# csteinmetz1/dasp-pytorch

Hardware: AMD Instinct MI355X
Metric: audio-samples/sec fwd+bwd, 6-band parametric_eq @ (256,2,131072) (higher is better)
Workload: dtype f32; 1 GPU; parametric_eq fwd+bwd (grad x + 18 controls) on (256,2,131072) fp32 per GPU, sr 44100, controls ~ U(ParametricEQ ranges); global_batch=256, parallelism=batch-shard x1, no collective, launch=eager, world_size=1

## Files before the change

dasp_pytorch_amd/csrc/sosfilt.hip:

```cpp
#include "common.hpp"
#include <type_traits>

#include "sos_tile.hpp"
#include <cstdlib>

namespace dasp {

__device__ __forceinline__ void nmul(double k, double p1, double q1, double p2, double q2, double& p, double& q) {
    p = p1 * p2 - k * q1 * q2;
    q = p1 * q2 + q1 * p2;
}
__device__ __forceinline__ void put_blk(float* o, double p, double q, double kap, int adj) {
    o[0] = (float)p;
    o[1] = (float)(adj ? -kap * q : q);
    o[2] = (float)(adj ? q : -kap * q);
    o[3] = (float)p;
}

struct D1 {
    double v, d;
};
__device__ __forceinline__ D1 dconst(double c) { return {c, 0.0}; }
__device__ __forceinline__ D1 operator+(D1 a, D1 b) { return {a.v + b.v, a.d + b.d}; }
__device__ __forceinline__ D1 operator-(D1 a, D1 b) { return {a.v - b.v, a.d - b.d}; }
__device__ __forceinline__ D1 operator*(D1 a, D1 b) { return {a.v * b.v, a.d * b.v + a.v * b.d}; }
__device__ __forceinline__ D1 operator/(D1 a, D1 b) {
    const double iv = 1.0 / b.v, q = a.v * iv;
    return {q, (a.d - q * b.d) * iv};
}
__device__ __forceinline__ D1 operator*(double c, D1 a) { return {c * a.v, c * a.d}; }
__device__ __forceinline__ D1 operator+(double c, D1 a) { return {c + a.v, a.d}; }
__device__ __forceinline__ D1 operator-(double c, D1 a) { return {c - a.v, -a.d}; }
__device__ __forceinline__ D1 operator-(D1 a) { return {-a.v, -a.d}; }
__device__ __forceinline__ D1 dsin(D1 a) { return {sin(a.v), cos(a.v) * a.d}; }
__device__ __forceinline__ D1 dcos(D1 a) { return {cos(a.v), -sin(a.v) * a.d}; }
__device__ __forceinline__ D1 dsqrt(D1 a) { const double r = sqrt(a.v); return {r, 0.5 / r * a.d}; }
__device__ __forceinline__ D1 dexp(D1 a) { const double e = exp(a.v); return {e, e * a.d}; }

struct PeqSpec {
    int types[8];
    double sample_rate;
    const float* rows[24];
    int norm;
    double lo[24], span[24];
    unsigned* flag;
};

__device__ void rbj_design(int type, double sample_rate, double gain_db, double fc, double qf, int dir, double* c5, double* dc5) {
    const D1 g = {gain_db, dir == 0 ? 1.0 : 0.0}, f = {fc, dir == 1 ? 1.0 : 0.0}, q = {qf, dir == 2 ? 1.0 : 0.0};
    const D1 A = dexp((2.302585092994045684 / 40.0) * g);
    const D1 w0 = (2.0 * 3.14159265358979323846 / sample_rate) * f;
    double sn, cs;
    sincos(w0.v, &sn, &cs);
    const D1 sw = {sn, cs * w0.d}, cw = {cs, -sn * w0.d};
    const D1 alpha = sw / (2.0 * q);
    const D1 sA = dsqrt(A);
    D1 b0, b1, b2, a0, a1, a2;
    if (type == 2) {
        b0 = A * ((A + dconst(1)) + (A - dconst(1)) * cw + 2.0 * (sA * alpha));
        b1 = -2.0 * (A * ((A - dconst(1)) + (A + dconst(1)) * cw));
        b2 = A * ((A + dconst(1)) + (A - dconst(1)) * cw - 2.0 * (sA * alpha));
        a0 = (A + dconst(1)) - (A - dconst(1)) * cw + 2.0 * (sA * alpha);
        a1 = 2.0 * ((A - dconst(1)) - (A + dconst(1)) * cw);
        a2 = (A + dconst(1)) - (A - dconst(1)) * cw - 2.0 * (sA * alpha);
    } else if (type == 1) {
        b0 = A * ((A + dconst(1)) - (A - dconst(1)) * cw + 2.0 * (sA * alpha));
        b1 = 2.0 * (A * ((A - dconst(1)) - (A + dconst(1)) * cw));
        b2 = A * ((A + dconst(1)) - (A - dconst(1)) * cw - 2.0 * (sA * alpha));
        a0 = (A + dconst(1)) + (A - dconst(1)) * cw + 2.0 * (sA * alpha);
        a1 = -2.0 * ((A - dconst(1)) + (A + dconst(1)) * cw);
        a2 = (A + dconst(1)) + (A - dconst(1)) * cw - 2.0 * (sA * alpha);
    } else if (type == 0) {
        b0 = 1.0 + alpha * A;
        b1 = -2.0 * cw;
        b2 = 1.0 - alpha * A;
        a0 = 1.0 + alpha / A;
        a1 = -2.0 * cw;
        a2 = 1.0 - alpha / A;
    } else if (type == 3) {
        b0 = 0.5 * (1.0 - cw);
        b1 = 1.0 - cw;
        b2 = 0.5 * (1.0 - cw);
        a0 = 1.0 + alpha;
        a1 = -2.0 * cw;
        a2 = 1.0 - alpha;
    } else {
        b0 = 0.5 * (1.0 + cw);
        b1 = -(1.0 + cw);
        b2 = 0.5 * (1.0 + cw);
        a0 = 1.0 + alpha;
        a1 = -2.0 * cw;
        a2 = 1.0 - alpha;
    }
    const D1 n[5] = {b0 / a0, b1 / a0, b2 / a0, a1 / a0, a2 / a0};
    for (int c = 0; c < 5; ++c) {
        c5[c] = n[c].v;
        dc5[c] = n[c].d;
    }
}

constexpr double OM_MIN = 1e-5;
#ifndef DASP_DF_OM_MIN
#define DASP_DF_OM_MIN 0.125
#endif
#ifndef DASP_STATES_CACHED
#define DASP_STATES_CACHED 1
#endif

template <int S>
__device__ __forceinline__ void section_coefs(const float* __restrict__ sos, const float* __restrict__ params, const PeqSpec& spec, int item, int k, int dir,
                                              bool report_range, double (&c5)[5], double (&dc5)[5], double& a0) {
    a0 = 1.0;
#pragma unroll
    for (int c = 0; c < 5; ++c) dc5[c] = 0.0;
    if (params && spec.norm) {
        const float* p = params + ((size_t)item * S + k) * 3;
        double v[3];
        for (int c = 0; c < 3; ++c) {
            const double pc = (double)p[c];
            if (report_range && spec.flag && (pc < 0.0 || pc > 1.0) && dir == 0) atomicOr(spec.flag, 1u << (3 * k + c));
            v[c] = spec.lo[3 * k + c] + spec.span[3 * k + c] * pc;
        }
        rbj_design(spec.types[k], spec.sample_rate, v[0], v[1], v[2], dir, c5, dc5);
        for (int c = 0; c < 5; ++c) dc5[c] *= spec.span[3 * k + dir];
    } else if (params) {
        const float* p = params + ((size_t)item * S + k) * 3;
        rbj_design(spec.types[k], spec.sample_rate, (double)p[0], (double)p[1], (double)p[2], dir, c5, dc5);
    } else if (!sos) {
        rbj_design(spec.types[k], spec.sample_rate, (double)spec.rows[3 * k][item], (double)spec.rows[3 * k + 1][item],
                   (double)spec.rows[3 * k + 2][item], dir, c5, dc5);
    } else {
        const float* sr = sos + ((size_t)item * S + k) * 6;
        a0 = (double)sr[3];
        c5[0] = sr[0] / a0; c5[1] = sr[1] / a0; c5[2] = sr[2] / a0; c5[3] = sr[4] / a0; c5[4] = sr[5] / a0;
    }
}

template <int S> struct GramFin;
template <int S, bool AGENT> __device__ __forceinline__ void gram_basis_responses(const double* cf, double* bas, int tid);
template <int S> __device__ __forceinline__ constexpr int basis_doubles();

template <int S, int L>
__global__ void __launch_bounds__(256)
sos_prep_kernel(const float* __restrict__ sos, const float* __restrict__ params, PeqSpec spec,
                float* __restrict__ tab, double* __restrict__ dtab, int nsq_seg = 0, double* __restrict__ segtab = nullptr,
                double* __restrict__ basis = nullptr, int nitems = 0) {
    using LY = SosLayout<S, L>;
    constexpr int S2 = 2 * S, NN = S2 * S2;
    __shared__ double sec[S][10];
    __shared__ double cfb[S][8];
    __shared__ double Phi[2][NN], T1[2][NN], T2[2][NN];
    __shared__ double vv[2][2][S2];
    if (basis && (int)blockIdx.x >= nitems) {
        const int it = blockIdx.x - nitems;
#ifdef DASP_TRACE
        if (it == 0 && threadIdx.x == 0) g_trace[48] = clock64();
#endif
        if (threadIdx.x < S) {
            double c5[5], dc5[5], a0;
            section_coefs<S>(sos, params, spec, it, threadIdx.x, 0, false, c5, dc5, a0);
            const double sg = -0.5 * c5[3];
            double om = sqrt(fabs(sg * sg - c5[4]));
            om = om < OM_MIN ? OM_MIN : om;
            for (int c = 0; c < 5; ++c) cfb[threadIdx.x][c] = c5[c];
            cfb[threadIdx.x][5] = sg; cfb[threadIdx.x][6] = om; cfb[threadIdx.x][7] = 1.0 / om;
        }
        __syncthreads();
#ifdef DASP_TRACE
        if (it == 0 && threadIdx.x == 0) g_trace[49] = clock64();
#endif
        gram_basis_responses<S, false>(&cfb[0][0], basis + (size_t)it * basis_doubles<S>(), threadIdx.x);
#ifdef DASP_TRACE
        asm volatile("s_waitcnt vmcnt(0)" ::: "memory");
        if (it == 0 && threadIdx.x == 0) g_trace[50] = clock64();
#endif
        return;
    }
    __shared__ float Gsh[2][L][S2];
    __shared__ double Pd[S][7][2];
    __shared__ float hsh[L];
    const int tid = threadIdx.x, item = blockIdx.x;
    PTRACE(40, 0);
    float* tb = tab + (size_t)item * LY::TOTAL;
    double* dt = dtab + (size_t)item * S * DT_STRIDE;

    if (tid < 4) tb[LY::CNT + tid] = 0.f;
    if (tid == 4) {
        const unsigned tg = ((unsigned)wall_clock64() * 2654435761u) ^ ((unsigned)item * 0x9E3779B1u);
        tb[LY::TAG] = __builtin_bit_cast(float, tg | 1u);
    }
    for (int e = tid; e < 2 * L * LY::YMC; e += 256) tb[LY::YM + e] = 0.f;
    if (tid < 3 * S) {
        const int k = tid / 3, dir = tid % 3;
        double c5[5], dc5[5], a0;
        section_coefs<S>(sos, params, spec, item, k, dir, true, c5, dc5, a0);
        double* d = dt + k * DT_STRIDE;
        for (int c = 0; c < 5; ++c) d[DT_J + c * 3 + dir] = dc5[c];
        if (dir == 0) {
            const double b0 = c5[0], b1 = c5[1], b2 = c5[2], a1 = c5[3], a2 = c5[4];
            const double sg = -0.5 * a1, disc = sg * sg - a2;
            const double kap = disc < 0 ? 1.0 : -1.0;
            double om = sqrt(fabs(disc));
            om = om < OM_MIN ? OM_MIN : om;
            const double g1 = b1 - b0 * a1, g2 = ((b2 - b0 * a2) + g1 * sg) / om;
            sec[k][0] = sg; sec[k][1] = om; sec[k][2] = kap * om; sec[k][3] = g1; sec[k][4] = g2; sec[k][5] = b0; sec[k][6] = kap;
            sec[k][7] = b1; sec[k][8] = b2;
            const bool direct = disc < 0 && om >= DASP_DF_OM_MIN && !(b0 == 1.0 && b1 == a1 && b2 == a2);
            float* df = tb + LY::DF + k * 8;
            df[0] = (float)b1; df[1] = (float)b2; df[2] = (float)-a1; df[3] = (float)-a2;
            df[4] = (float)(-g1 * sg + g2 * om); df[5] = (float)(-g1 * kap * om - g2 * sg); df[6] = (float)(1.0 / om); df[7] = (float)(sg / om);
            float* cf = tb + LY::COEF + k * 8;
            cf[0] = (float)sg; cf[1] = (float)om; cf[2] = (float)(kap * om); cf[3] = (float)g1; cf[4] = (float)g2;
            cf[5] = (float)b0; cf[6] = (float)kap; cf[7] = direct ? 1.f : 0.f;
            d[DT_OM] = direct ? 1.0 : om;
            for (int c = 0; c < 5; ++c) d[DT_B0 + c] = c5[c];
            d[DT_A0] = a0; d[7] = kap;
            d[23] = 0.0;
            d[DT_SG32] = (double)(float)sg; d[DT_NF] = direct ? 0.0 : 1.0; d[27] = 0.0;
        }
    }
    PTRACE(41, 0);
    __syncthreads();
    PTRACE(47, 0);
    for (int e = tid; e < 2 * NN; e += 256) {
        const int sys = e / NN, i = (e % NN) / S2, j = e % S2;
        const int kk = i / 2, r = i % 2, jj = j / 2, c = j % 2;
        const int fk = sys ? S - 1 - kk : kk, fj = sys ? S - 1 - jj : jj;
        const double sg = sec[fk][0], om = sec[fk][1], kom = sec[fk][2];
        const int rr = sys ? c : r, cc = sys ? r : c;
        const double a_el = rr == cc ? sg : (rr == 0 ? -kom : om);
        const double Bk = sys ? sec[fk][3 + r] : (r == 0 ? 1.0 : 0.0);
        const double Cj = sys ? (c == 0 ? 1.0 : 0.0) : sec[fj][3 + c];
        double gain = 1.0;
#pragma unroll
        for (int m = 0; m < S; ++m) {
            const double dm = sec[sys ? S - 1 - m : m][5];
            gain *= (m > jj && m < kk) ? dm : 1.0;
        }
        const double v = jj == kk ? a_el : (jj < kk ? Bk * gain * Cj : 0.0);
        Phi[sys][i * S2 + j] = v;
        T1[sys][i * S2 + j] = v;
        T2[sys][i * S2 + j] = 0.0;
    }
    PTRACE(46, 0);
    if (tid < 2 * S2) {
        const int sys = tid / S2, i = tid % S2, kk = i / 2, r = i % 2;
        const int fk = sys ? S - 1 - kk : kk;
        double gain = 1.0;
        for (int m = 0; m < kk; ++m) gain *= sec[sys ? S - 1 - m : m][5];
        vv[0][sys][i] = (sys ? sec[fk][3 + r] : (r == 0 ? 1.0 : 0.0)) * gain;
    }
    PTRACE(42, 0);
    __syncthreads();

    if (tid < 64) {
        for (int m = 0; m < L; ++m) {
            const int cur = m & 1;
            if (tid < 2 * S2) {
                const int sys = tid / S2, i = tid % S2;
                const double v = vv[cur][sys][i];
                Gsh[sys][m][i] = (float)v;
                double acc = 0.0;
                for (int j = 0; j < S2; ++j) acc += Phi[sys][i * S2 + j] * vv[cur][sys][j];
                vv[cur ^ 1][sys][i] = acc;
            }
            wave_lds_sync();
        }
    } else if (tid >= 128 && tid < 128 + 1 + S2) {
        const int ex = tid - 128, c0 = ex - 1;
        double s1[S], s2[S];
#pragma unroll
        for (int k = 0; k < S; ++k) { s1[k] = (c0 == 2 * k) ? 1.0 : 0.0; s2[k] = (c0 == 2 * k + 1) ? 1.0 : 0.0; }
        for (int n = 0; n < L; ++n) {
            double u = (ex == 0 && n == 0) ? 1.0 : 0.0;
#pragma unroll
            for (int k = 0; k < S; ++k) {
                const double sg = sec[k][0], om = sec[k][1], kom = sec[k][2], g1 = sec[k][3], g2 = sec[k][4], d = sec[k][5];
                const double o = d * u + g1 * s1[k] + g2 * s2[k];
                const double t1 = sg * s1[k] - kom * s2[k] + u;
                s2[k] = om * s1[k] + sg * s2[k];
                s1[k] = t1;
                u = o;
            }
            if (ex == 0) hsh[n] = (float)u;
            else tb[LY::YM + n * LY::YMC + L + state_pos<S>(c0)] = (float)u;
        }
    } else if (tid >= 192 && tid < 192 + S2) {
        const int c0 = tid - 192;
        double l1[S], l2[S];
#pragma unroll
        for (int i = 0; i < S; ++i) { l1[i] = (c0 == 2 * i) ? 1.0 : 0.0; l2[i] = (c0 == 2 * i + 1) ? 1.0 : 0.0; }
        for (int n = L - 1; n >= 0; --n) {
            double g = 0.0;
#pragma unroll
            for (int i = 0; i < S; ++i) {
                const int k = S - 1 - i;
                const double sg = sec[k][0], om = sec[k][1], kom = sec[k][2], g1 = sec[k][3], g2 = sec[k][4], d = sec[k][5];
                const double o = d * g + l1[i];
                const double t1 = sg * l1[i] + om * l2[i] + g1 * g;
                l2[i] = -kom * l1[i] + sg * l2[i] + g2 * g;
                l1[i] = t1;
                g = o;
            }
            tb[LY::YMA + n * LY::YMC + L + state_pos<S>(c0)] = (float)g;
        }
    } else if (tid < 128) {
        const int l = tid - 64;
        double (*src)[NN] = T1;
        double (*dst)[NN] = T2;
        for (int step = 1; step < L; step <<= 1) {
            constexpr int NTRI = S * (S + 1) / 2 * 4;
            for (int e = l; e < 2 * NTRI; e += 64) {
                const int sys = e / NTRI, q = e % NTRI, blk = q >> 2;
                const int kk = (blk >= 1) + (blk >= 3) + (blk >= 6) + (blk >= 10) + (blk >= 15) + (blk >= 21) + (blk >= 28);
                const int jj = blk - kk * (kk + 1) / 2;
                const int i = 2 * kk + ((q >> 1) & 1), j = 2 * jj + (q & 1);
                double acc = 0.0;
#pragma unroll
                for (int m = 0; m < S2; ++m) acc += src[sys][i * S2 + m] * src[sys][m * S2 + j];
                dst[sys][i * S2 + j] = acc;
            }
            wave_lds_sync();
            double (*tmp)[NN] = src; src = dst; dst = tmp;
        }
        for (int e = l; e < 2 * S * S * 4; e += 64) {
            const int sys = e / (S * S * 4), k = (e / (S * 4)) % S, j = (e / 4) % S, c = e % 4;
            tb[(sys ? LY::MCA : LY::MC) + (k * S + j) * 4 + c] = (float)src[sys][(2 * k + (c & 1)) * S2 + 2 * j + (c >> 1)];
        }
        if (l < S) {
            const int k = l;
            const double kap = sec[k][6];
            double p = src[0][(2 * k) * S2 + 2 * k], q = src[0][(2 * k + 1) * S2 + 2 * k];
            for (int lv = 0; lv < 7; ++lv) {
                Pd[k][lv][0] = p; Pd[k][lv][1] = q;
                if (lv < 4) {
                    put_blk(tb + LY::PL + (k * 4 + lv) * 4, p, q, kap, 0);
                    put_blk(tb + LY::PLA + ((S - 1 - k) * 4 + lv) * 4, p, q, kap, 1);
                }
                if (lv == 6) {
                    put_blk(tb + LY::P64 + k * 4, p, q, kap, 0);
                    put_blk(tb + LY::P64A + (S - 1 - k) * 4, p, q, kap, 1);
                }
                double p2, q2;
                nmul(kap, p, q, p, q, p2, q2);
                p = p2; q = q2;
            }
        }
    }
    PTRACE(43, 0); PTRACE(44, 64);
    __syncthreads();
    for (int e = tid; e < L * L; e += 256) {
        const int n = e / L, j = e % L;
        if (j <= n) tb[LY::YM + n * LY::YMC + j] = hsh[n - j];
        else tb[LY::YMA + n * LY::YMC + j] = hsh[j - n];
        if (j == n) tb[LY::YMA + n * LY::YMC + j] = hsh[0];
    }
    for (int e = tid; e < 2 * L * S2; e += 256) {
        const int sys = e / (L * S2), m = (e / S2) % L, i = e % S2;
        if (sys == 0) tb[LY::GT + ((i >> 1) * L + (L - 1 - m)) * 2 + (i & 1)] = Gsh[0][m][i];
        else tb[LY::GAT + ((i >> 1) * L + m) * 2 + (i & 1)] = Gsh[1][m][i];
    }
    for (int e = tid; e < S * 64; e += 256) {
        const int k = e / 64, c = e % 64, m = c + 1;
        const double kap = sec[k][6];
        double p = 1.0, q = 0.0;
        for (int l = 0; l < 7; ++l)
            if (m & (1 << l)) {
                double p2, q2;
                nmul(kap, p, q, Pd[k][l][0], Pd[k][l][1], p2, q2);
                p = p2; q = q2;
            }
        put_blk(tb + LY::PW + (k * 64 + c) * 4, p, q, kap, 0);
        put_blk(tb + LY::PWA + ((S - 1 - k) * 64 + c) * 4, p, q, kap, 1);
    }
    PTRACE(45, 0);
    if (segtab) {
        constexpr int NTRI = S * (S + 1) / 2 * 4;
        int nl = 0;
        for (int v = L; v > 1; v >>= 1) ++nl;
        double (*src)[NN] = (nl & 1) ? T2 : T1;
        double (*dst)[NN] = (nl & 1) ? T1 : T2;
        for (int step = 0; step < nsq_seg; ++step) {
            for (int e = tid; e < 2 * NTRI; e += 256) {
                const int sys = e / NTRI, q = e % NTRI, blk = q >> 2;
                const int kk = (blk >= 1) + (blk >= 3) + (blk >= 6) + (blk >= 10) + (blk >= 15) + (blk >= 21) + (blk >= 28);
                const int jj = blk - kk * (kk + 1) / 2;
                const int i = 2 * kk + ((q >> 1) & 1), j = 2 * jj + (q & 1);
                double acc = 0.0;
#pragma unroll
                for (int m = 0; m < S2; ++m) acc += src[sys][i * S2 + m] * src[sys][m * S2 + j];
                dst[sys][i * S2 + j] = acc;
            }
            __syncthreads();
            double (*tmp)[NN] = src; src = dst; dst = tmp;
        }
        for (int e = tid; e < 2 * NN; e += 256) segtab[(size_t)item * 2 * NN + e] = src[e / NN][e % NN];
    }
}

__device__ __forceinline__ void seg_state_store(float* p, f2 v) {
    __hip_atomic_store(p, v.x, __ATOMIC_RELAXED, __HIP_MEMORY_SCOPE_AGENT);
    __hip_atomic_store(p + 1, v.y, __ATOMIC_RELAXED, __HIP_MEMORY_SCOPE_AGENT);
}
template <int S, int W>
__device__ __forceinline__ void chain_by_last_workgroup(int* __restrict__ cnt, int n_wg, const double* __restrict__ Phi, const float* z,
                                                        float* __restrict__ start, int row0, int nrows, int G, int adjoint,
                                                        float* __restrict__ scratch , int scratch_stride) {
    constexpr int S2 = 2 * S, GB = 64;
    __shared__ int s_last;
    __shared__ double s_st[W][2][S2];
    asm volatile("s_waitcnt vmcnt(0)" ::: "memory");
    __syncthreads();
    if (threadIdx.x == 0) {
        s_last = handoff_arrive_is_last(cnt, n_wg);
    }
    __syncthreads();
    if (!s_last) return;
    const int l = lane_id(), w = wave_id();
    float* zs = scratch + w * scratch_stride;
    double prow[S2];
#pragma unroll
    for (int j = 0; j < S2; ++j) prow[j] = l < S2 ? Phi[l * S2 + j] : 0.0;
    const int first = adjoint ? G - 1 : 0, step = adjoint ? -1 : 1;
    for (int row = row0 + w; row < row0 + nrows; row += W) {
        if (l < S2) {
            s_st[w][0][l] = 0.0;
            start[((size_t)row * G + first) * S2 + l] = 0.f;
        }
        int cur = 0;
        for (int n0 = 0; n0 < G - 1; n0 += GB) {
            const int nblk = G - 1 - n0 < GB ? G - 1 - n0 : GB;
            wave_lds_sync();
            for (int e = l; e < nblk * S2; e += 64) {
                const int g = first + (n0 + e / S2) * step;
                zs[e] = __hip_atomic_load(z + ((size_t)row * G + g) * S2 + e % S2, __ATOMIC_RELAXED, __HIP_MEMORY_SCOPE_AGENT);
            }
            wave_lds_sync();
            for (int i = 0; i < nblk; ++i) {
                const int g = first + (n0 + i) * step;
                if (l < S2) {
                    double acc = (double)zs[i * S2 + l];
#pragma unroll
                    for (int j = 0; j < S2; ++j) acc += prow[j] * s_st[w][cur][j];
                    s_st[w][cur ^ 1][l] = acc;
                    start[((size_t)row * G + g + step) * S2 + l] = (float)acc;
                }
                wave_lds_sync();
                cur ^= 1;
            }
        }
    }
}


__device__ __forceinline__ void lookback_publish(unsigned long long* w, float v, unsigned tag) {
    __hip_atomic_store(w, ((unsigned long long)tag << 32) | __builtin_bit_cast(unsigned, v), __ATOMIC_RELAXED, __HIP_MEMORY_SCOPE_AGENT);
}
template <int S, int W>
__device__ __forceinline__ void lookback_start(const unsigned long long* z64, int seg, int G, int order, const double* __restrict__ Phi, unsigned tag,
                                               float* inbox, int seq, float* zs ,
                                               double (*st)[2 * S] , unsigned* err, int family) {
    constexpr int S2 = 2 * S, GB = 64;
    const int l = lane_id(), w = wave_id();
    const int npred = order > 0 ? seg : G - 1 - seg, first = order > 0 ? 0 : G - 1;
    double prow[S2];
#pragma unroll
    for (int j = 0; j < S2; ++j) prow[j] = w == 0 && l < S2 && npred > 0 ? Phi[l * S2 + j] : 0.0;
    if (w == 0 && l < S2) st[0][l] = 0.0;
    int cur = 0;
    __syncthreads();
    for (int n0 = 0; n0 < npred; n0 += GB) {
        const int nblk = npred - n0 < GB ? npred - n0 : GB;
        if (n0) __syncthreads();
        for (int e = threadIdx.x; e < nblk * S2; e += 64 * W) {
            const unsigned long long* wp = z64 + (size_t)(first + order * (n0 + e / S2)) * S2 + e % S2;
            zs[e] = lookback_poll(wp, tag, err, family);
        }
        __syncthreads();
        if (w == 0) {
            for (int i = 0; i < nblk; ++i) {
                if (l < S2) {
                    double acc = (double)zs[i * S2 + l];
#pragma unroll
                    for (int j = 0; j < S2; ++j) acc += prow[j] * st[cur][j];
                    st[cur ^ 1][l] = acc;
                }
                wave_lds_sync();
                cur ^= 1;
            }
        }
    }
    if (w == 0) {
        wave_lds_sync();
        if (l < S2) inbox[4 * (l >> 1) + (l & 1)] = (float)st[cur][l];
        if (l < S) inbox[4 * l + 2] = __builtin_bit_cast(float, seq);
    }
}

template <int S, int L, int W, int SEG = 0>
__global__ void __launch_bounds__(64 * W, W >= 16 ? 4 : (W * 2 + 3) / 4)
sos_fwd_kernel(const float* __restrict__ tab, int tab_bcast, const float* __restrict__ x, float* __restrict__ y,
               float* __restrict__ carries, int C, int N, int nt, int vec,
               int G = 1, int Tseg = 0, const float* __restrict__ segstart = nullptr, float* __restrict__ zseg = nullptr,
               float* __restrict__ chain_tab = nullptr, const double* __restrict__ segtab = nullptr, float* __restrict__ chain_start = nullptr,
               unsigned* __restrict__ err = nullptr) {
    using LY = SosLayout<S, L>;
    constexpr int S2 = 2 * S, TS = 64 * L, IMG = 64 * L;
    constexpr int LDS_T = W * 2 * IMG, LDS_MB = W * S * 4, LDS_PW = S * 64 * 4;
    __shared__ __attribute__((aligned(16))) float lds[LDS_T + LDS_MB + LDS_PW];
    const int lane = lane_id(), wave = wave_id();
    const int row = SEG ? blockIdx.x / G : blockIdx.x, seg = SEG ? blockIdx.x % G : 0;
    const int t0 = SEG ? seg * Tseg : 0, t1 = SEG ? (t0 + Tseg < nt ? t0 + Tseg : nt) : nt;
    const float* __restrict__ tb = tab + (size_t)(tab_bcast ? 0 : row / C) * LY::TOTAL;
    const float* __restrict__ xr = x + (size_t)row * N;
    float* __restrict__ yr = y + (size_t)row * N;
    const int mb_in = wave * S * 4, mb_out = ((wave + 1) % W) * S * 4;
    float* pw_lds = lds + LDS_MB;
    float* tbx = pw_lds + LDS_PW + wave * 2 * IMG;
    float* tby = tbx + IMG;
    if (SEG) {
        for (int i = threadIdx.x; i < LDS_MB; i += 64 * W) {
            float v = 0.f;
            if (i < S * 4) {
                const int comp = i & 3;
                if (comp == 2) v = __builtin_bit_cast(float, t0);
                else if (SEG == 1 && comp < 2) v = segstart[((size_t)row * G + seg) * S2 + 2 * (i >> 2) + comp];
            }
            lds[i] = v;
        }
    } else {
        for (int i = threadIdx.x; i < LDS_MB; i += 64 * W) lds[i] = 0.f;
    }
    for (int i = threadIdx.x; i < LDS_PW; i += 64 * W) pw_lds[i] = tb[LY::PW + i];
    __syncthreads();
    const f4* pws = reinterpret_cast<const f4*>(pw_lds);

    f2 Kreg[S];
#pragma unroll
    for (int k = 0; k < S; ++k) Kreg[k] = f2{0.f, 0.f};
    const unsigned a_x = __builtin_amdgcn_readfirstlane(lds_addr(tbx));
    float Aop[4];
    chunk_table_operands<S, L>(tb + LY::GT, Aop, lane);
    static_assert(L == 16 && S2 <= 16, "one 16 x 16 output block per 16 chunks");
    float AT[4], AO[4];
    if (SEG != 2) cascade_map_operands<S, L>(tb + LY::YM, LY::YMC, AT, AO, lane);
    const unsigned tag = SEG == 3 ? __builtin_amdgcn_readfirstlane(__builtin_bit_cast(unsigned, tb[LY::TAG])) : 0u;
    unsigned long long* z64 = reinterpret_cast<unsigned long long*>(zseg) + (size_t)row * G * S2;

    auto sweep = [&](auto scan_tag, const int seq0, const bool first_tile_requested = false) {
        constexpr bool SCAN = decltype(scan_tag)::value;
        if (!first_tile_requested && t0 + wave < t1 && tile_full<L>((long)(t0 + wave) * TS, N, vec)) tile_dma_issue_swz(xr + (size_t)(t0 + wave) * TS, a_x, lane);
        int stores_in_flight = 0;
        for (int t = t0 + wave; t < t1; t += W) {
            int toff = 0;
            asm volatile("" : "+s"(toff));
            const float* __restrict__ tbl = tb + toff;
            const bool full = tile_full<L>((long)t * TS, N, vec);
            WIDE_PRIO(DASP_SCAN_PRIO);
            TRACE(0);
            if (full) wait_vmcnt(stores_in_flight);
            else tile_global_to_swz_guarded(tbx, xr, (long)t * TS, N);
            f4 Bop[4], zacc[4];
            chunk_products_load(tbx, Bop, lane);
            pin(Bop);
            if (t + W < t1 && tile_full<L>((long)(t + W) * TS, N, vec)) tile_dma_issue_swz(xr + (size_t)(t + W) * TS, a_x, lane);
            TRACE(1);
            float Z[L];
            chunk_products_issue(Bop, Aop, zacc);
            chunk_products_collect<L>(tby, zacc, Z, lane, lane);
            pin(Z); TRACE(5);

            f2 st[S];
            MboxPeek pk;
            SCAN_PRIO(DASP_SCAN_PRIO);
            tile_scan<S, L>(Z, [](f2 v) { return v; }, st, tbl + LY::MC, tbl + LY::PL, tbl + LY::P64, pws, lane,
                [&](int k) { if (W > 1) pk = mbox_peek(lds, mb_in + 4 * k); },
                [&](int k, f2& K) {
                    if (W == 1) K = Kreg[k];
                    else if (pk.seq == t + seq0) K = f2{pk.a, pk.b};
                    else { float a, b; mbox_wait(lds, mb_in + 4 * k, t + seq0, a, b); K = f2{a, b}; }
                },
                [&](int k, f2 Kn) {
                    if (W == 1) Kreg[k] = f2{read_lane(Kn.x, 63), read_lane(Kn.y, 63)};
                    else if (t + 1 < t1) mbox_publish<63>(lds, mb_out + 4 * k, Kn.x, Kn.y, t + 1 + seq0);
                    else if (SCAN && lane == 63) {
                        if (SEG == 3) { lookback_publish(z64 + (size_t)seg * S2 + 2 * k, Kn.x, tag); lookback_publish(z64 + (size_t)seg * S2 + 2 * k + 1, Kn.y, tag); }
                        else seg_state_store(zseg + ((size_t)row * G + seg) * S2 + 2 * k, Kn);
                    }
                }
#ifdef DASP_TRACE
                , blockIdx.x == 7 && threadIdx.x == 64 && t >= 40 && t < 40 + W
#endif
                );
            SCAN_PRIO(0);
            TRACE(2);
            if (SCAN) {
                stores_in_flight = 0;
                continue;
            }
            if (carries) {
                static_assert(S % 2 == 0, "states are stored in section pairs");
                f4* cs = reinterpret_cast<f4*>(carries) + ((size_t)row * nt + t) * (S / 2) * 64 + lane;
#pragma unroll
                for (int m = 0; m < S / 2; ++m) {
                    const f4 v = f4{st[2 * m].x, st[2 * m].y, st[2 * m + 1].x, st[2 * m + 1].y};
                    if (DASP_FWD_NT & 4) st_stream(cs + m * 64, v); else cs[m * 64] = v;
                }
            }

            f4 yacc[4];
            cascade_outputs_mfma_acc<S, L>(tby, st, Bop, AT, AO, lane, yacc);
            TRACE(3);
            WIDE_PRIO(DASP_SCAN_PRIO);
            if (DASP_DIRECT_OUT && full) {
                mfma_granules_to_global(yr + (size_t)t * TS, yacc, DASP_FWD_NT & 2, lane);
            } else {
                mfma_granules_to_image(tby, yacc, lane);
                if (full) tile_swz_to_global_full(tby, yr, (long)t * TS, DASP_FWD_NT & 2, lane);
                else tile_swz_to_global_guarded(tby, yr, (long)t * TS, N);
            }
            stores_in_flight = full ? (carries ? S / 2 : 0) + L / 4 : -1;
            TRACE(4);
        }
    };
    if (SEG == 3) {
        sweep(std::true_type{}, 0);
        constexpr int SEQ2 = 1 << 28;
        __shared__ double lb_st[2][S2];
        if (t0 + wave < t1 && tile_full<L>((long)(t0 + wave) * TS, N, vec)) tile_dma_issue_swz(xr + (size_t)(t0 + wave) * TS, a_x, lane);
        lookback_start<S, W>(z64, seg, G, 1, segtab + (size_t)(tab_bcast ? 0 : row / C) * 2 * S2 * S2, tag, lds, t0 + SEQ2, pw_lds + LDS_PW + IMG, lb_st, err, DASP_DEVERR_SOS_FWD);
        __syncthreads();
        sweep(std::false_type{}, SEQ2, true);
    } else if (SEG == 2) {
        sweep(std::true_type{}, 0);
    } else {
        sweep(std::false_type{}, 0);
    }
    if (SEG == 2 && chain_tab) {
        const int item = tab_bcast ? 0 : row / C;
        chain_by_last_workgroup<S, W>(reinterpret_cast<int*>(chain_tab + (size_t)item * LY::TOTAL + LY::CNT) + 1, tab_bcast ? (int)gridDim.x : C * G,
                                      segtab + (size_t)item * 2 * S2 * S2, zseg, chain_start, tab_bcast ? 0 : item * C,
                                      tab_bcast ? (int)gridDim.x / G : C, G, 0, pw_lds + LDS_PW, 2 * IMG);
    }
}

#include "sos_gram_fin.hpp"

template <int S, int L, int W, int SEG = 0>
__global__ void __launch_bounds__(64 * W, (W * 2 + 3) / 4)
sos_bwd_kernel(const float* __restrict__ tab, int tab_bcast, const float* __restrict__ gy, float* __restrict__ gx, int C, int N, int nt, int vec,
               int G = 1, int Tseg = 0, const float* __restrict__ segstart = nullptr, float* __restrict__ zseg = nullptr,
               float* __restrict__ chain_tab = nullptr, const double* __restrict__ segtab = nullptr, float* __restrict__ chain_start = nullptr) {
    using LY = SosLayout<S, L>;
    constexpr bool GX = SEG != 2;
    constexpr int S2 = 2 * S, TS = 64 * L, IMG = 64 * L, REGION = 2 * IMG;
    constexpr int LDS_T = W * REGION, LDS_MB = W * S * 4, LDS_PW = S * 64 * 4, LDS_CF = S * 16;
    __shared__ __attribute__((aligned(16))) float lds[LDS_T + LDS_MB + LDS_PW + LDS_CF];
    const int lane = lane_id(), wave = wave_id();
    const int row = SEG ? blockIdx.x / G : blockIdx.x, seg = SEG ? blockIdx.x % G : 0;
    const int t0 = SEG ? seg * Tseg : 0, t1 = SEG ? (t0 + Tseg < nt ? t0 + Tseg : nt) : nt, nr = t1 - t0;
    const float* __restrict__ tb = tab + (size_t)(tab_bcast ? 0 : row / C) * LY::TOTAL;
    const float* __restrict__ gr = gy + (size_t)row * N;
    float* __restrict__ gxr = gx + (size_t)row * N;
    const int mb_in = wave * S * 4, mb_out = ((wave + 1) % W) * S * 4;
    float* cf_lds = lds + LDS_MB;
    float* pw_lds = cf_lds + LDS_CF;
    float* tbg = pw_lds + LDS_PW + wave * REGION;
    float* tbo = tbg + IMG;
    for (int i = threadIdx.x; i < LDS_MB; i += 64 * W) {
        float v = 0.f;
        if (i < S * 4) {
            const int comp = i & 3;
            if (comp == 2) v = __builtin_bit_cast(float, t1);
            else if (SEG == 1 && comp < 2) v = segstart[((size_t)row * G + seg) * S2 + 2 * (i >> 2) + comp];
        }
        lds[i] = v;
    }
    for (int i = threadIdx.x; i < LDS_PW; i += 64 * W) pw_lds[i] = tb[LY::PWA + i];
    for (int i = threadIdx.x; i < S * 8; i += 64 * W) cf_lds[i] = tb[LY::COEF + i];
    for (int i = threadIdx.x; i < S * 8; i += 64 * W) cf_lds[S * 8 + i] = tb[LY::DF + i];
// ... 927 lines not shown
```

Before: 192.0 billion channel-samples/s.

## Restructure sos prep kernel to overlap per-wave table writes and drop a barrier

```diff
diff --git a/dasp_pytorch_amd/csrc/sosfilt.hip b/dasp_pytorch_amd/csrc/sosfilt.hip
--- a/dasp_pytorch_amd/csrc/sosfilt.hip
+++ b/dasp_pytorch_amd/csrc/sosfilt.hip
@@ -146,7 +146,7 @@
                 float* __restrict__ tab, double* __restrict__ dtab, int nsq_seg = 0, double* __restrict__ segtab = nullptr,
                 double* __restrict__ basis = nullptr, int nitems = 0) {
     using LY = SosLayout<S, L>;
-    constexpr int S2 = 2 * S, NN = S2 * S2;
+    constexpr int S2 = 2 * S, NN = S2 * S2, NTRI = S * (S + 1) / 2 * 4;
     __shared__ double sec[S][10];
     __shared__ double cfb[S][8];
     __shared__ double Phi[2][NN], T1[2][NN], T2[2][NN];
@@ -190,6 +190,7 @@
         tb[LY::TAG] = __builtin_bit_cast(float, tg | 1u);
     }
     for (int e = tid; e < 2 * L * LY::YMC; e += 256) tb[LY::YM + e] = 0.f;
+    for (int e = tid; e < 2 * NN; e += 256) { (&Phi[0][0])[e] = 0.0; (&T1[0][0])[e] = 0.0; (&T2[0][0])[e] = 0.0; }
     if (tid < 3 * S) {
         const int k = tid / 3, dir = tid % 3;
         double c5[5], dc5[5], a0;
@@ -222,9 +223,11 @@
     PTRACE(41, 0);
     __syncthreads();
     PTRACE(47, 0);
-    for (int e = tid; e < 2 * NN; e += 256) {
-        const int sys = e / NN, i = (e % NN) / S2, j = e % S2;
-        const int kk = i / 2, r = i % 2, jj = j / 2, c = j % 2;
+    for (int e = tid; e < 2 * NTRI; e += 256) {
+        const int sys = e / NTRI, q = e % NTRI, blk = q >> 2;
+        const int kk = (blk >= 1) + (blk >= 3) + (blk >= 6) + (blk >= 10) + (blk >= 15) + (blk >= 21) + (blk >= 28);
+        const int jj = blk - kk * (kk + 1) / 2;
+        const int r = (q >> 1) & 1, c = q & 1, i = 2 * kk + r, j = 2 * jj + c;
         const int fk = sys ? S - 1 - kk : kk, fj = sys ? S - 1 - jj : jj;
         const double sg = sec[fk][0], om = sec[fk][1], kom = sec[fk][2];
         const int rr = sys ? c : r, cc = sys ? r : c;
@@ -237,79 +240,136 @@
             const double dm = sec[sys ? S - 1 - m : m][5];
             gain *= (m > jj && m < kk) ? dm : 1.0;
         }
-        const double v = jj == kk ? a_el : (jj < kk ? Bk * gain * Cj : 0.0);
+        const double v = jj == kk ? a_el : Bk * gain * Cj;
         Phi[sys][i * S2 + j] = v;
         T1[sys][i * S2 + j] = v;
-        T2[sys][i * S2 + j] = 0.0;
     }
     PTRACE(46, 0);
-    if (tid < 2 * S2) {
-        const int sys = tid / S2, i = tid % S2, kk = i / 2, r = i % 2;
+    if (tid >= 192 && tid < 192 + 2 * S2) {
+        const int t3 = tid - 192, sys = t3 / S2, i = t3 % S2, kk = i / 2, r = i % 2;
         const int fk = sys ? S - 1 - kk : kk;
         double gain = 1.0;
-        for (int m = 0; m < kk; ++m) gain *= sec[sys ? S - 1 - m : m][5];
+#pragma unroll
+        for (int m = 0; m < S; ++m) {
+            const double dm = sec[sys ? S - 1 - m : m][5];
+            gain *= m < kk ? dm : 1.0;
+        }
         vv[0][sys][i] = (sys ? sec[fk][3 + r] : (r == 0 ? 1.0 : 0.0)) * gain;
     }
+    PTRACE(37, 192);
+    if (tid >= 192 && tid < 192 + S) {
+        const int k = tid - 192;
+        const double kap = sec[k][6];
+        double m00 = sec[k][0], m01 = -sec[k][2], m10 = sec[k][1], m11 = sec[k][0];
+        for (int step = 1; step < L; step <<= 1) {
+            double n00 = 0.0, n01 = 0.0, n10 = 0.0, n11 = 0.0;
+            n00 += m00 * m00; n00 += m01 * m10;
+            n01 += m00 * m01; n01 += m01 * m11;
+            n10 += m10 * m00; n10 += m11 * m10;
+            n11 += m10 * m01; n11 += m11 * m11;
+            m00 = n00; m01 = n01; m10 = n10; m11 = n11;
+        }
+        double p = m00, q = m10;
+        for (int lv = 0; lv < 7; ++lv) {
+            Pd[k][lv][0] = p; Pd[k][lv][1] = q;
+            double p2, q2;
+            nmul(kap, p, q, p, q, p2, q2);
+            p = p2; q = q2;
+        }
+    }
+    PTRACE(38, 192);
     PTRACE(42, 0);
     __syncthreads();
 
     if (tid < 64) {
+        const int sys = tid < S2 ? 0 : 1, i = tid < 2 * S2 ? tid - sys * S2 : 0;
+        double prow[S2];
+#pragma unroll
+        for (int j = 0; j < S2; ++j) prow[j] = Phi[sys][i * S2 + j];
         for (int m = 0; m < L; ++m) {
             const int cur = m & 1;
             if (tid < 2 * S2) {
-                const int sys = tid / S2, i = tid % S2;
                 const double v = vv[cur][sys][i];
                 Gsh[sys][m][i] = (float)v;
                 double acc = 0.0;
-                for (int j = 0; j < S2; ++j) acc += Phi[sys][i * S2 + j] * vv[cur][sys][j];
+#pragma unroll
+                for (int j = 0; j < S2; ++j) acc += prow[j] * vv[cur][sys][j];
                 vv[cur ^ 1][sys][i] = acc;
             }
             wave_lds_sync();
         }
-    } else if (tid >= 128 && tid < 128 + 1 + S2) {
+        PTRACE(43, 0);
+        for (int e = tid; e < 2 * L * S2; e += 64) {
+            const int sys = e / (L * S2), m = (e / S2) % L, i = e % S2;
+            if (sys == 0) tb[LY::GT + ((i >> 1) * L + (L - 1 - m)) * 2 + (i & 1)] = Gsh[0][m][i];
+            else tb[LY::GAT + ((i >> 1) * L + m) * 2 + (i & 1)] = Gsh[1][m][i];
+        }
+    } else if (tid >= 128 && tid < 192) {
         const int ex = tid - 128, c0 = ex - 1;
-        double s1[S], s2[S];
-#pragma unroll
-        for (int k = 0; k < S; ++k) { s1[k] = (c0 == 2 * k) ? 1.0 : 0.0; s2[k] = (c0 == 2 * k + 1) ? 1.0 : 0.0; }
-        for (int n = 0; n < L; ++n) {
-            double u = (ex == 0 && n == 0) ? 1.0 : 0.0;
-#pragma unroll
-            for (int k = 0; k < S; ++k) {
-                const double sg = sec[k][0], om = sec[k][1], kom = sec[k][2], g1 = sec[k][3], g2 = sec[k][4], d = sec[k][5];
-                const double o = d * u + g1 * s1[k] + g2 * s2[k];
-                const double t1 = sg * s1[k] - kom * s2[k] + u;
-                s2[k] = om * s1[k] + sg * s2[k];
-                s1[k] = t1;
-                u = o;
-            }
-            if (ex == 0) hsh[n] = (float)u;
-            else tb[LY::YM + n * LY::YMC + L + state_pos<S>(c0)] = (float)u;
-        }
-    } else if (tid >= 192 && tid < 192 + S2) {
+        if (ex < 1 + S2) {
+            double s1[S], s2[S];
+#pragma unroll
+            for (int k = 0; k < S; ++k) { s1[k] = (c0 == 2 * k) ? 1.0 : 0.0; s2[k] = (c0 == 2 * k + 1) ? 1.0 : 0.0; }
+            for (int n = 0; n < L; ++n) {
+                double u = (ex == 0 && n == 0) ? 1.0 : 0.0;
+#pragma unroll
+                for (int k = 0; k < S; ++k) {
+                    const double sg = sec[k][0], om = sec[k][1], kom = sec[k][2], g1 = sec[k][3], g2 = sec[k][4], d = sec[k][5];
+                    const double o = d * u + g1 * s1[k] + g2 * s2[k];
+                    const double t1 = sg * s1[k] - kom * s2[k] + u;
+                    s2[k] = om * s1[k] + sg * s2[k];
+                    s1[k] = t1;
+                    u = o;
+                }
+                if (ex == 0) hsh[n] = (float)u;
+                else tb[LY::YM + n * LY::YMC + L + state_pos<S>(c0)] = (float)u;
+            }
+        }
+        PTRACE(32, 128);
+        wave_lds_sync();
+        for (int e = ex; e < L * L; e += 64) {
+            const int n = e / L, j = e % L;
+            if (j <= n) tb[LY::YM + n * LY::YMC + j] = hsh[n - j];
+            else tb[LY::YMA + n * LY::YMC + j] = hsh[j - n];
+            if (j == n) tb[LY::YMA + n * LY::YMC + j] = hsh[0];
+        }
+    } else if (tid >= 192) {
         const int c0 = tid - 192;
-        double l1[S], l2[S];
-#pragma unroll
-        for (int i = 0; i < S; ++i) { l1[i] = (c0 == 2 * i) ? 1.0 : 0.0; l2[i] = (c0 == 2 * i + 1) ? 1.0 : 0.0; }
-        for (int n = L - 1; n >= 0; --n) {
-            double g = 0.0;
-#pragma unroll
-            for (int i = 0; i < S; ++i) {
-                const int k = S - 1 - i;
-                const double sg = sec[k][0], om = sec[k][1], kom = sec[k][2], g1 = sec[k][3], g2 = sec[k][4], d = sec[k][5];
-                const double o = d * g + l1[i];
-                const double t1 = sg * l1[i] + om * l2[i] + g1 * g;
-                l2[i] = -kom * l1[i] + sg * l2[i] + g2 * g;
-                l1[i] = t1;
-                g = o;
-            }
-            tb[LY::YMA + n * LY::YMC + L + state_pos<S>(c0)] = (float)g;
-        }
-    } else if (tid < 128) {
+        if (c0 < S2) {
+            double l1[S], l2[S];
+#pragma unroll
+            for (int i = 0; i < S; ++i) { l1[i] = (c0 == 2 * i) ? 1.0 : 0.0; l2[i] = (c0 == 2 * i + 1) ? 1.0 : 0.0; }
+            for (int n = L - 1; n >= 0; --n) {
+                double g = 0.0;
+#pragma unroll
+                for (int i = 0; i < S; ++i) {
+                    const int k = S - 1 - i;
+                    const double sg = sec[k][0], om = sec[k][1], kom = sec[k][2], g1 = sec[k][3], g2 = sec[k][4], d = sec[k][5];
+                    const double o = d * g + l1[i];
+                    const double t1 = sg * l1[i] + om * l2[i] + g1 * g;
+                    l2[i] = -kom * l1[i] + sg * l2[i] + g2 * g;
+                    l1[i] = t1;
+                    g = o;
+                }
+                tb[LY::YMA + n * LY::YMC + L + state_pos<S>(c0)] = (float)g;
+            }
+        }
+        PTRACE(33, 192);
+        if (c0 < S) {
+            const int k = c0;
+            const double kap = sec[k][6];
+            for (int lv = 0; lv < 4; ++lv) {
+                put_blk(tb + LY::PL + (k * 4 + lv) * 4, Pd[k][lv][0], Pd[k][lv][1], kap, 0);
+                put_blk(tb + LY::PLA + ((S - 1 - k) * 4 + lv) * 4, Pd[k][lv][0], Pd[k][lv][1], kap, 1);
+            }
+            put_blk(tb + LY::P64 + k * 4, Pd[k][6][0], Pd[k][6][1], kap, 0);
+            put_blk(tb + LY::P64A + (S - 1 - k) * 4, Pd[k][6][0], Pd[k][6][1], kap, 1);
+        }
+    } else {
         const int l = tid - 64;
         double (*src)[NN] = T1;
         double (*dst)[NN] = T2;
         for (int step = 1; step < L; step <<= 1) {
-            constexpr int NTRI = S * (S + 1) / 2 * 4;
             for (int e = l; e < 2 * NTRI; e += 64) {
                 const int sys = e / NTRI, q = e % NTRI, blk = q >> 2;
                 const int kk = (blk >= 1) + (blk >= 3) + (blk >= 6) + (blk >= 10) + (blk >= 15) + (blk >= 21) + (blk >= 28);
@@ -323,59 +383,40 @@
             wave_lds_sync();
             double (*tmp)[NN] = src; src = dst; dst = tmp;
         }
+        PTRACE(30, 64);
         for (int e = l; e < 2 * S * S * 4; e += 64) {
             const int sys = e / (S * S * 4), k = (e / (S * 4)) % S, j = (e / 4) % S, c = e % 4;
             tb[(sys ? LY::MCA : LY::MC) + (k * S + j) * 4 + c] = (float)src[sys][(2 * k + (c & 1)) * S2 + 2 * j + (c >> 1)];
         }
-        if (l < S) {
-            const int k = l;
+        PTRACE(44, 64);
+    }
+    if (tid < 64 || tid >= 128) {
+        constexpr int N3 = (S + 1) / 2, N2 = (S - N3 + 1) / 2;
+        const int c = tid & 63, m = c + 1;
+        const int k0 = tid >= 192 ? 0 : (tid >= 128 ? N3 : N3 + N2), k1 = tid >= 192 ? N3 : (tid >= 128 ? N3 + N2 : S);
+        for (int k = k0; k < k1; ++k) {
             const double kap = sec[k][6];
-            double p = src[0][(2 * k) * S2 + 2 * k], q = src[0][(2 * k + 1) * S2 + 2 * k];
-            for (int lv = 0; lv < 7; ++lv) {
-                Pd[k][lv][0] = p; Pd[k][lv][1] = q;
-                if (lv < 4) {
-                    put_blk(tb + LY::PL + (k * 4 + lv) * 4, p, q, kap, 0);
-                    put_blk(tb + LY::PLA + ((S - 1 - k) * 4 + lv) * 4, p, q, kap, 1);
-                }
-                if (lv == 6) {
-                    put_blk(tb + LY::P64 + k * 4, p, q, kap, 0);
-                    put_blk(tb + LY::P64A + (S - 1 - k) * 4, p, q, kap, 1);
-                }
+            double pd[7][2];
+#pragma unroll
+            for (int l = 0; l < 7; ++l) { pd[l][0] = Pd[k][l][0]; pd[l][1] = Pd[k][l][1]; }
+            double p = 1.0, q = 0.0;
+#pragma unroll
+            for (int l = 0; l < 7; ++l) {
                 double p2, q2;
-                nmul(kap, p, q, p, q, p2, q2);
-                p = p2; q = q2;
-            }
-        }
-    }
-    PTRACE(43, 0); PTRACE(44, 64);
+                nmul(kap, p, q, pd[l][0], pd[l][1], p2, q2);
+                p = (m & (1 << l)) ? p2 : p; q = (m & (1 << l)) ? q2 : q;
+            }
+            put_blk(tb + LY::PW + (k * 64 + c) * 4, p, q, kap, 0);
+            put_blk(tb + LY::PWA + ((S - 1 - k) * 64 + c) * 4, p, q, kap, 1);
+        }
+    }
+    PTRACE(34, 0); PTRACE(35, 128); PTRACE(36, 192);
+#ifdef DASP_TRACE
     __syncthreads();
-    for (int e = tid; e < L * L; e += 256) {
-        const int n = e / L, j = e % L;
-        if (j <= n) tb[LY::YM + n * LY::YMC + j] = hsh[n - j];
-        else tb[LY::YMA + n * LY::YMC + j] = hsh[j - n];
-        if (j == n) tb[LY::YMA + n * LY::YMC + j] = hsh[0];
-    }
-    for (int e = tid; e < 2 * L * S2; e += 256) {
-        const int sys = e / (L * S2), m = (e / S2) % L, i = e % S2;
-        if (sys == 0) tb[LY::GT + ((i >> 1) * L + (L - 1 - m)) * 2 + (i & 1)] = Gsh[0][m][i];
-        else tb[LY::GAT + ((i >> 1) * L + m) * 2 + (i & 1)] = Gsh[1][m][i];
-    }
-    for (int e = tid; e < S * 64; e += 256) {
-        const int k = e / 64, c = e % 64, m = c + 1;
-        const double kap = sec[k][6];
-        double p = 1.0, q = 0.0;
-        for (int l = 0; l < 7; ++l)
-            if (m & (1 << l)) {
-                double p2, q2;
-                nmul(kap, p, q, Pd[k][l][0], Pd[k][l][1], p2, q2);
-                p = p2; q = q2;
-            }
-        put_blk(tb + LY::PW + (k * 64 + c) * 4, p, q, kap, 0);
-        put_blk(tb + LY::PWA + ((S - 1 - k) * 64 + c) * 4, p, q, kap, 1);
-    }
+#endif
     PTRACE(45, 0);
     if (segtab) {
-        constexpr int NTRI = S * (S + 1) / 2 * 4;
+        __syncthreads();
         int nl = 0;
         for (int v = L; v > 1; v >>= 1) ++nl;
         double (*src)[NN] = (nl & 1) ? T2 : T1;
```

Result: no change. 192.4 billion channel-samples/s, median of 3 (+0.2%).
